# dontLoveBugs/CSPN_monodepth

Hardware: AMD Instinct MI355X
Metric: depth-maps/sec at 304x228 b=24, 24 CSPN iters (higher is better)
Workload: dtype f32

## Files before the change

### cspn_monodepth_amd/csrc/cspn_resident.hip

```cpp
#include "cspn_common.hpp"

#include <atomic>

namespace {

struct ResArgs {
    const float* g;
    long g_bs, g_cs;
    const float* d0;
    const float* sparse;
    float* out;
    float* xbuf;
    unsigned* flags;
    unsigned* status;
    unsigned* host_err;
    int last_chunk;
    unsigned seq;
    float* hist;
    float* w_out;
    float* s_out;
    const float* s_in;
    const float* target;
    double* macc;
    int nslots;
    int B, H, W, Wv, T, S;
    int tw, th, tiles_x, tiles_y;
    int wq, wr, hxw, hyw, dr, ls;
    int b0, nb;
    unsigned spin_limit;
    unsigned long long* dbg;
};

__device__ __forceinline__ void st4_dev(float* base, unsigned elem, float a, float b, float c, float d) {
    const v4f v = {a, b, c, d};
    asm volatile("global_store_dwordx4 %0, %1, %2 sc1" ::"v"(elem * 4u), "v"(v), "s"(base) : "memory");
}
template <typename T>
__device__ __forceinline__ T* uniform_ptr(T* p) {
    const unsigned long long u = reinterpret_cast<unsigned long long>(p);
    const unsigned lo = __builtin_amdgcn_readfirstlane((unsigned)u), hi = __builtin_amdgcn_readfirstlane((unsigned)(u >> 32));
    return reinterpret_cast<T*>(((unsigned long long)hi << 32) | lo);
}
#define GLB __attribute__((address_space(1)))
typedef GLB char* gptr;
__device__ __forceinline__ gptr at32(const float* base, unsigned e) {
    return (gptr) reinterpret_cast<unsigned long long>(base) + (e << 2);
}
__device__ __forceinline__ float4 ld4(gptr p) {
    const v4f v = *reinterpret_cast<const GLB v4f*>(p);
    return make_float4(v.x, v.y, v.z, v.w);
}
__device__ __forceinline__ float ld1(gptr p) { return *reinterpret_cast<const GLB float*>(p); }
__device__ __forceinline__ void st4(gptr p, float4 v) {
// ... 5 lines not shown
#endif
#ifndef CSPN_RES_STEP_PIPE
#define CSPN_RES_STEP_PIPE 0
#endif
#ifndef CSPN_RES_PUBLISH_ALL
#define CSPN_RES_PUBLISH_ALL 1
#endif
__device__ __forceinline__ void st4_hist(gptr p, float4 v) {
    const v4f w = {v.x, v.y, v.z, v.w};
    if (CSPN_RES_HIST_NT) __builtin_nontemporal_store(w, reinterpret_cast<GLB v4f*>(p));
    else *reinterpret_cast<GLB v4f*>(p) = w;
}
__device__ __forceinline__ float4 ld4_dev(gptr p) {
    const unsigned long long lo = __hip_atomic_load(reinterpret_cast<const GLB unsigned long long*>(p), __ATOMIC_RELAXED, __HIP_MEMORY_SCOPE_AGENT);
    const unsigned long long hi = __hip_atomic_load(reinterpret_cast<const GLB unsigned long long*>(p) + 1, __ATOMIC_RELAXED, __HIP_MEMORY_SCOPE_AGENT);
    return make_float4(__uint_as_float((unsigned)lo), __uint_as_float((unsigned)(lo >> 32)), __uint_as_float((unsigned)hi),
                       __uint_as_float((unsigned)(hi >> 32)));
}
__device__ __forceinline__ float ld1_dev(gptr p) {
    return __uint_as_float(__hip_atomic_load(reinterpret_cast<const GLB unsigned*>(p), __ATOMIC_RELAXED, __HIP_MEMORY_SCOPE_AGENT));
}

constexpr int RES_THREADS = 512;
constexpr int RES_PP = 16352;

template <int NQ, int NTHREADS, int BLEND, int MODE, int CLEAN, int PAC = 0>
__global__ __launch_bounds__(NTHREADS, NTHREADS / 256) void cspn3_resident(const ResArgs a) {
    static_assert(!PAC || MODE <= 2, "the softmax-weight form has no transposed sweep of its own (the published volume feeds MODE 3)");
    constexpr int R = 1, NT = 8, WIN = 6;
    constexpr bool SCORE = MODE == 1, TRANSG = MODE == 4, TRANS = MODE == 3 || TRANSG, HIST = MODE == 2 || TRANS;
    extern __shared__ __attribute__((aligned(16))) float lds[];
    __shared__ int wg_bad;

    const int tid = threadIdx.x;
    const int tiles_per_img = a.tiles_x * a.tiles_y;
    const int wg_round = a.nb * tiles_per_img;
    const int round = (int)blockIdx.x / wg_round;
    const int tile = xcd_contiguous_id((int)blockIdx.x - round * wg_round, wg_round);
    const int bl = tile / tiles_per_img;
    const int trem = tile - bl * tiles_per_img;
    const int ty = trem / a.tiles_x;
    const int tx = trem - ty * a.tiles_x;
    const int b = a.b0 + round * a.nb + bl;
    const int H = a.H, W = a.W;
    const int y0 = ty * a.th, x0 = tx * a.tw;
    const size_t HW = (size_t)H * W;
    const size_t plane = (size_t)a.B * HW;
    if (tid == 0) wg_bad = 0;
    int n_stamp = 0;
    auto stamp = [&]() { if (a.dbg && tid == 0 && round == 0 && n_stamp < 16) a.dbg[(size_t)blockIdx.x * 16 + n_stamp++] = wall_clock64(); };
    stamp();
    auto count_out = [&]() {
        if (HIST && tid == 0) {
            const unsigned old = __hip_atomic_fetch_add(a.status + 2, 1u, __ATOMIC_RELAXED, __HIP_MEMORY_SCOPE_AGENT);
            if (old + 1u == gridDim.x) {
                __hip_atomic_store(a.status + 2, 0u, __ATOMIC_RELAXED, __HIP_MEMORY_SCOPE_AGENT);
                if (a.host_err && a.last_chunk) __hip_atomic_store(a.host_err + 1, a.seq, __ATOMIC_RELAXED, __HIP_MEMORY_SCOPE_SYSTEM);
            }
        }
    };

    if (b >= a.B) { count_out(); return; }

    const float* __restrict__ din0 = uniform_ptr(a.d0 + (size_t)b * HW);
    const float* __restrict__ spg = BLEND ? uniform_ptr(a.sparse + (size_t)b * HW) : nullptr;

    const int wq = a.wq, wr = a.wr;
    const int sy = tid / wq;
    const int sx = tid - sy * wq;
    const int r0 = sy * NQ;
    const bool exch = a.T > a.S;
    const int rx0 = max(exch ? max(0, x0 - a.tw) : 0, min(x0 - a.hxw, W - 4 * wq));
    const int ry0 = max(exch ? max(0, y0 - a.th) : 0, min(y0 - a.hyw, H - wr));
    const int xq = rx0 + 4 * sx;
    const int yq0 = ry0 + r0;
    const bool x_in = (xq >= 0) && (xq < a.Wv);
    const int nval = a.Wv - xq;
    const int lane = tid & 63;
    const bool fix_left = (sx == 0) || (lane == 0);
    const bool fix_right = (sx == wq - 1) || (lane == 63);

    const int dr = a.dr, ls = a.ls;
    float* const cur = lds;
    float* const nxt = lds + RES_PP;
    const int yd0 = ry0 - R;
    const int xd0 = rx0 - 4;
    float4 st0[NQ + 1];
    unsigned st0_in = 0;
    const int step_r = NTHREADS / wq, step_q = NTHREADS - step_r * wq;
    {
    int row = sy, qx = sx;
#pragma unroll
    for (int u = 0; u <= NQ; ++u) {
        const int y = yd0 + row, x = xd0 + 4 + 4 * qx;
        const bool valid = row < dr;
        const bool in = valid && (y >= 0 && y < H && x >= 0 && x < a.Wv);
// ... 23 lines not shown
    float* const md_lds = lds + RES_PP + (size_t)a.dr * a.ls;
    const float* __restrict__ gq = uniform_ptr(a.g + (size_t)b * a.g_bs);
    float edge[NQ][6];
    const unsigned ucs = (unsigned)a.g_cs;
    float srow[TRANSG ? NQ + 2 : 1][6];
    if constexpr (TRANSG) {
        const float* __restrict__ sq = uniform_ptr(a.s_in + (size_t)b * HW);
#pragma unroll
        for (int m = 0; m < NQ + 2; ++m) {
            const int ys = yq0 - 1 + m;
            const bool v = x_in && ys >= 0 && ys < H;
            const unsigned o = v ? (unsigned)(ys * W + xq) : 0u;
            const float4 q4 = ld4(at32(sq, o));
            srow[m][0] = q4.x; srow[m][1] = q4.y; srow[m][2] = q4.z; srow[m][3] = q4.w;
            srow[m][4] = ld1(at32(sq, (v && fix_left && xq >= 1) ? o - 1u : 0u));
            srow[m][5] = ld1(at32(sq, (v && fix_right && xq + 4 < a.Wv) ? o + 4u : 0u));
        }
    }
#pragma unroll
    for (int i = 0; i < NQ; ++i) {
        const int r = r0 + i, y = yq0 + i;
        const bool ok = (r < wr) && x_in && (y >= 0) && (y < H);
        if (ok) in_img |= 1u << i;
        if (ok && y >= y0 && y < y0 + a.th && xq >= x0 && xq < x0 + a.tw) interior |= 1u << i;
        unsigned orow[3];
        bool rokv[3];
#pragma unroll
        for (int d = 0; d < 3; ++d) {
            const int row = y + d - 1;
            rokv[d] = ok && row >= 0 && row < H;
            orow[d] = rokv[d] ? (unsigned)(row * W + xq) : 0u;
        }
#pragma unroll
        for (int j = 0; j < NT; ++j) {
            const int lin = j < 4 ? j : j + 1;
            const int d = (PAC || TRANSG) ? 1 : lin / 3;
            const float4 v = ld4(at32(gq, (unsigned)((PAC || TRANSG) ? j : 7 - j) * ucs + orow[d]));
            wreg[i][j][0] = rokv[d] ? v.x : 0.f; wreg[i][j][1] = rokv[d] ? v.y : 0.f;
            wreg[i][j][2] = rokv[d] ? v.z : 0.f; wreg[i][j][3] = rokv[d] ? v.w : 0.f;
        }
#pragma unroll
        for (int t = 0; t < 6; ++t) edge[i][t] = 0.f;
        if (!PAC && !TRANSG && (fix_left || fix_right)) {
#pragma unroll
            for (int t = 0; t < 6; ++t) {
                const bool lft = t < 3;
                const int j = lft ? (t == 0 ? 0 : (t == 1 ? 3 : 5)) : (t == 3 ? 2 : (t == 4 ? 4 : 7));
// ... 148 lines not shown
        }
    }

    stamp();
    int r0L = r0, sxL = sx, yq0L = yq0, xqL = xq;
    asm volatile("" : "+v"(r0L), "+v"(sxL), "+v"(yq0L), "+v"(xqL));
    const bool active = (r0L < wr);
    const int cb = 4 + 4 * sxL;
    float* __restrict__ dout = HIST ? nullptr : uniform_ptr(a.out + (size_t)b * HW);
    float* hist_step = HIST ? uniform_ptr(a.hist + (size_t)b * HW) : nullptr;
    const int n_phase = (a.T + a.S - 1) / a.S;
    const int tile_global = b * tiles_per_img + trem;
    float own[NQ][4];
    float nbl[NQ], nbr[NQ];

    for (int p = 0; p < n_phase; ++p) {
        const int steps = (a.T - p * a.S) < a.S ? (a.T - p * a.S) : a.S;
        const bool last_phase = (p == n_phase - 1);
        const float* __restrict__ xin = uniform_ptr(a.xbuf + (size_t)((p + 1) & 1) * plane + (size_t)b * HW);
        if (p > 0) {
            int tidp = tid;
            asm volatile("" : "+v"(tidp));
            const int tq_in = min(a.tw, rx0 + 4 * wq - x0) >> 2;
            const int th_in = min(a.th, ry0 + wr - y0);
            const int nl = (x0 - rx0) >> 2;
            const int nside = wq - tq_in;
            const int nrow_t = (y0 - ry0) + R;
            const int n_top = nrow_t * wq;
            const int n_bot = (dr - nrow_t - th_in) * wq;
            const int n_side = th_in * nside;
            const int n_halo = n_top + n_bot + n_side;
            float ring_v = 0.f;
            int ring_at = -1;
            if (tidp < dr * 2 * R) {
                const int row = tidp / (2 * R), c = tidp - row * (2 * R);
                const int lc = (c < R) ? (4 - R + c) : (4 + 4 * wq + (c - R));
                const int y = yd0 + row, x = xd0 + lc;
                const bool in = (y >= 0 && y < H && x >= 0 && x < a.Wv);
                const float v = ld1_dev(at32(xin, in ? (unsigned)(y * W + x) : 0u));
                ring_v = in ? v : 0.f;
                ring_at = row * ls + lc;
            }
            for (int base = 0; base < n_halo; base += 2 * NTHREADS) {
                float4 hv[2];
                int at[2];
#pragma unroll
                for (int u = 0; u < 2; ++u) {
// ... 189 lines not shown
        stamp();
        const int plain_steps = last_phase ? steps - 1 : steps;
        using P0 = std::integral_constant<int, 0>;
        using P1 = std::integral_constant<int, 1>;
        if (__ballot(active) != 0ull) {
            int s = 0;
            for (; s + 1 < plain_steps; s += 2) {
                step(std::false_type{}, std::true_type{}, P0{}, 0);
                step(std::false_type{}, std::true_type{}, P1{}, 0);
            }
            if (s < plain_steps) step(std::false_type{}, std::true_type{}, P0{}, 0);
            if (last_phase) step(std::true_type{}, std::true_type{}, P0{}, plain_steps & 1);
        } else {
            for (int s = 0; s < plain_steps; ++s) step(std::false_type{}, std::false_type{}, P0{}, 0);
            if (last_phase) step(std::true_type{}, std::false_type{}, P0{}, 0);
        }
        stamp();
        if (!last_phase) {
            float* __restrict__ xout = uniform_ptr(a.xbuf + (size_t)(p & 1) * plane + (size_t)b * HW);
            if (active) {
                unsigned o0 = (unsigned)(yq0L * W + xqL);
                asm volatile("" : "+v"(o0));
#if !CSPN_RES_PUBLISH_ALL
                auto reg_x0 = [&](int t) { const int xx0 = t * a.tw; return max(max(0, xx0 - a.tw), min(xx0 - a.hxw, W - 4 * wq)); };
                auto reg_y0 = [&](int t) { const int yy0 = t * a.th; return max(max(0, yy0 - a.th), min(yy0 - a.hyw, H - wr)); };
                const int pubL = tx > 0 ? reg_x0(tx - 1) + 4 * wq + 1 : -(1 << 30);
                const int pubR = tx + 1 < a.tiles_x ? reg_x0(tx + 1) - 1 : (1 << 30);
                const int pubT = ty > 0 ? reg_y0(ty - 1) + wr + 1 : -(1 << 30);
                const int pubB = ty + 1 < a.tiles_y ? reg_y0(ty + 1) - 1 : (1 << 30);
                const bool col_read = (xqL < pubL) || (xqL + 3 >= pubR);
#endif
#pragma unroll
                for (int i = 0; i < NQ; ++i) {
#if !CSPN_RES_PUBLISH_ALL
                    const bool read = col_read || (yq0L + i < pubT) || (yq0L + i >= pubB);
#else
                    const bool read = true;
#endif
                    if (((interior >> i) & 1u) && read) st4_dev(xout, o0 + (unsigned)(i * W), own[i][0], own[i][1], own[i][2], own[i][3]);
                }
            }
            asm volatile("s_waitcnt vmcnt(0)" ::: "memory");
            __syncthreads();
            const unsigned want = a.seq + (unsigned)p + 1u;
            if (tid == 0) __hip_atomic_store(a.flags + tile_global, want, __ATOMIC_RELAXED, __HIP_MEMORY_SCOPE_AGENT);
            if (tid < 9 && tid != 4) {
                const int ny = ty + tid / 3 - 1, nx = tx + tid % 3 - 1;
                if (ny >= 0 && ny < a.tiles_y && nx >= 0 && nx < a.tiles_x) {
// ... 71 lines not shown
        }
        __syncthreads();
        if (tid < 10) {
            double v = 0.0;
            for (int w = 0; w < NTHREADS / 64; ++w) v += (double)part[w * 10 + tid];
            if (v != 0.0) atomicAdd(a.macc + (size_t)(blockIdx.x % a.nslots) * 10 + tid, v);
        }
    }
    count_out();
}

constexpr int RES_MAX_NQ = 5;

constexpr int RES_MAX_ROUNDS = 8;
#ifndef CSPN_RES_ONE_LAUNCH
#define CSPN_RES_ONE_LAUNCH 0
#endif
struct ResGeom {
    int S, tiles_x, tiles_y, tw, th, nq, wq, wr, hxw, hyw, dr, ls;
    int imgs_per_launch, launches;
    size_t lds_bytes;
    double cost;
    int threads = RES_THREADS;
};

int cu_count() {
    static std::atomic<int> cached[64];
    int dev = 0;
    if (hipGetDevice(&dev) != hipSuccess) return 0;
    int n = cached[dev & 63].load(std::memory_order_relaxed);
    if (n > 0) return n;
    hipDeviceProp_t prop;
    if (hipGetDeviceProperties(&prop, dev) != hipSuccess) return 0;
    cached[dev & 63].store(prop.multiProcessorCount, std::memory_order_relaxed);
    return prop.multiProcessorCount;
}

size_t res_lds_bytes(int dr, int ls, int nq, int blend, int threads = RES_THREADS) {
    return ((size_t)RES_PP + (size_t)dr * ls + (size_t)(blend ? 1 : 0) * threads * nq * 4 + 16 * 10) * sizeof(float);
}

#ifndef CSPN_RES_LS_SWIZZLE
#define CSPN_RES_LS_SWIZZLE 1
#endif
int res_row_stride(int wq, int nq, int dr) {
    const int lo = 4 * wq + 8;
    if (!CSPN_RES_LS_SWIZZLE) return lo;
    for (int cand = lo; cand < lo + 64; cand += 4)
        if ((((nq * cand - 4 * wq) % 64) + 64) % 64 == 0 && (size_t)dr * cand <= (size_t)RES_PP) return cand;
    return lo;
}

bool regions_inside_image(const ResGeom& g, int H, int W, int Wv, int T) {
    if (Wv != W) return false;
    const bool exch = T > g.S;
    for (int tx = 0; tx < g.tiles_x; ++tx) {
        const int x0 = tx * g.tw;
        int rx0 = x0 - g.hxw; if (rx0 > W - 4 * g.wq) rx0 = W - 4 * g.wq;
        int lo = exch ? x0 - g.tw : 0; if (lo < 0) lo = 0;
        if (rx0 < lo) rx0 = lo;
        if (rx0 + 4 * g.wq > W) return false;
    }
    for (int ty = 0; ty < g.tiles_y; ++ty) {
        const int y0 = ty * g.th;
        int ry0 = y0 - g.hyw; if (ry0 > H - g.wr) ry0 = H - g.wr;
        int lo = exch ? y0 - g.th : 0; if (lo < 0) lo = 0;
        if (ry0 < lo) ry0 = lo;
        if (ry0 + g.wr > H) return false;
    }
    return true;
}

bool resident_geometry(int B, int H, int W, int T, int blend, int ncu, int S_user, ResGeom* best, int threads = RES_THREADS) {
    if (W % 4 != 0 || ncu < 1 || T < 1) return false;
    if (threads != 1024) threads = RES_THREADS;
    const int max_nq = threads == 1024 ? 1 : RES_MAX_NQ;
    bool found = false;
    for (int S = (S_user > 0 ? S_user : 12); S >= (S_user > 0 ? S_user : 4); S -= (S > 8 ? 4 : 2)) {
        const int Se = S > T ? T : S;
        const int hyw = Se - 1, hxw = round_up4(Se - 1);
        const int phases = ceil_div(T, Se);
        if (phases > 1 && (Se & 1)) continue;
        for (int tx = 1; tx <= 32; ++tx) {
            const int tw = round_up4(ceil_div(W, tx));
            if (tx > 1 && (tw < 16 || ceil_div(W, tw) != tx)) continue;
            if (phases > 1 && tx > 1 && tw < 2 * hxw) continue;
            const int wq = (tw + 2 * hxw) / 4;
            if (wq > threads) continue;
            for (int ty = 1; ty <= 64; ++ty) {
                const int th = ceil_div(H, ty);
                if (ty > 1 && (th < 4 || ceil_div(H, th) != ty)) continue;
                if (phases > 1 && ty > 1 && th < 2 * hyw) continue;
                const int tiles = tx * ty;
                if (tiles > ncu) continue;
                const int wr = th + 2 * hyw;
                const int rows_per_thread_col = threads / wq;
                const int nq = ceil_div(wr, rows_per_thread_col);
                if (nq > max_nq) continue;
                const int dr = wr + 2, ls = res_row_stride(wq, nq, dr);
                if ((size_t)dr * ls > (size_t)RES_PP) continue;
                const size_t ldsb = res_lds_bytes(dr, ls, nq, blend, threads);
                if (ldsb > 160 * 1024) continue;
                int ipl = ncu / tiles;
                if (ipl > B) ipl = B;
                const int launches = ceil_div(B, ipl);
                ResGeom cand{Se, tx, ty, tw, th, nq, wq, wr, hxw, hyw, dr, ls, ipl, launches, ldsb, 0.0};
                const double pen = regions_inside_image(cand, H, W, W, T) ? 1.0 : 1.13;
                const double cost = launches * (8.0 + 2.0 * nq + T * (0.13 * nq + 0.1) * pen + (phases - 1) * (3.0 + 0.6 * nq));
                if (!found || cost < best->cost) {
                    found = true;
                    *best = ResGeom{Se, tx, ty, tw, th, nq, wq, wr, hxw, hyw, dr, ls, ipl, launches, ldsb, cost};
                    best->threads = threads;
                }
            }
        }
    }
    return found;
}

template <int NQ, int BLEND, int MODE, int CLEAN, int PAC = 0, int NTH = RES_THREADS>
int launch_resident_inst(const ResArgs& a, int grid, size_t lds_bytes, hipStream_t st) {
    constexpr auto kern = cspn3_resident<NQ, NTH, BLEND, MODE, CLEAN, PAC>;
    static std::atomic<size_t> granted[64];
    int dev = 0;
    HIP_OK(hipGetDevice(&dev));
    if (lds_bytes > 64 * 1024 && granted[dev & 63].load(std::memory_order_acquire) < lds_bytes) {
        HIP_OK(hipFuncSetAttribute(reinterpret_cast<const void*>(kern), hipFuncAttributeMaxDynamicSharedMemorySize, (int)lds_bytes));
        granted[dev & 63].store(lds_bytes, std::memory_order_release);
    }
    hipLaunchKernelGGL(kern, dim3(grid), dim3(NTH), lds_bytes, st, a);
    HIP_OK(hipGetLastError());
    return 1;
}

template <int CLEAN>
int launch_resident_1024(const ResArgs& a, int grid, size_t lds, int blend, int mode, hipStream_t st) {
    if (mode == 0) return blend ? launch_resident_inst<1, 1, 0, CLEAN, 0, 1024>(a, grid, lds, st) : launch_resident_inst<1, 0, 0, CLEAN, 0, 1024>(a, grid, lds, st);
    if (mode == 1) return blend ? launch_resident_inst<1, 1, 1, CLEAN, 0, 1024>(a, grid, lds, st) : launch_resident_inst<1, 0, 1, CLEAN, 0, 1024>(a, grid, lds, st);
    return fail("cspn3_forward_resident: 1024-thread workgroups serve the inference forms only");
}

template <int NQ, int CLEAN>
int launch_resident_c(const ResArgs& a, int grid, size_t lds, int blend, int mode, hipStream_t st) {
    if (mode >= 4 && mode <= 6) {
        if (mode == 6) return blend ? launch_resident_inst<NQ, 1, 2, CLEAN, 1>(a, grid, lds, st) : launch_resident_inst<NQ, 0, 2, CLEAN, 1>(a, grid, lds, st);
        if (blend) return mode == 5 ? launch_resident_inst<NQ, 1, 1, CLEAN, 1>(a, grid, lds, st) : launch_resident_inst<NQ, 1, 0, CLEAN, 1>(a, grid, lds, st);
        return mode == 5 ? launch_resident_inst<NQ, 0, 1, CLEAN, 1>(a, grid, lds, st) : launch_resident_inst<NQ, 0, 0, CLEAN, 1>(a, grid, lds, st);
    }
    if (mode == 7) return blend ? launch_resident_inst<NQ, 1, 4, CLEAN>(a, grid, lds, st) : launch_resident_inst<NQ, 0, 4, CLEAN>(a, grid, lds, st);
    if (mode == 3) return blend ? launch_resident_inst<NQ, 1, 3, CLEAN>(a, grid, lds, st) : launch_resident_inst<NQ, 0, 3, CLEAN>(a, grid, lds, st);
    if (blend) {
        if (mode == 2) return launch_resident_inst<NQ, 1, 2, CLEAN>(a, grid, lds, st);
        return mode ? launch_resident_inst<NQ, 1, 1, CLEAN>(a, grid, lds, st) : launch_resident_inst<NQ, 1, 0, CLEAN>(a, grid, lds, st);
    }
    if (mode == 2) return launch_resident_inst<NQ, 0, 2, CLEAN>(a, grid, lds, st);
    return mode ? launch_resident_inst<NQ, 0, 1, CLEAN>(a, grid, lds, st) : launch_resident_inst<NQ, 0, 0, CLEAN>(a, grid, lds, st);
}
template <int NQ>
int launch_resident_nq(const ResArgs& a, int grid, size_t lds, int blend, int mode, bool clean, hipStream_t st) {
    return clean ? launch_resident_c<NQ, 1>(a, grid, lds, blend, mode, st) : launch_resident_c<NQ, 0>(a, grid, lds, blend, mode, st);
}


}

namespace {
int resident_launch(const void* guidance, long bs, long cs, const void* d0, const void* sparse, void* out, void* history,
                    void* w8_out, float* s_out, void* work, unsigned seq, unsigned* host_err, int B, int H, int W, int W_valid,
                    int T, int blend, const void* target, double* acc, int nslots, const cspn_resident_plan* plan,
                    cspn_stream_t stream, bool transposed, bool pac = false, const float* s_in = nullptr);
}

extern "C" {

int cspn3_resident_plan(int B, int H, int W, int T, int blend, int n_cu, cspn_resident_plan* out) {
    if (!out || B < 1 || H < 1 || W < 1 || T < 0) return fail("cspn3_resident_plan: bad arguments");
    if (n_cu <= 0) n_cu = cu_count();
    if (n_cu <= 0) return fail("cspn3_resident_plan: no device (pass n_cu > 0 to plan without one)");
    ResGeom g;
    if (T < 1 || !resident_geometry(B, H, W, T, blend, n_cu, out->steps_per_phase, &g, out->threads))
        return fail("cspn3_resident_plan: no resident tiling for B=%d %dx%d T=%d on %d CUs (W %% 4 == 0 needed)", B, H, W, T, n_cu);
    if (ceil_div(T, g.S) > 255) return fail("cspn3_resident_plan: T=%d in %d-step phases is more than 255 phases", T, g.S);
    out->steps_per_phase = g.S; out->tiles_x = g.tiles_x; out->tiles_y = g.tiles_y; out->tile_w = g.tw; out->tile_h = g.th;
    out->quads_per_thread = g.nq; out->threads = g.threads; out->images_per_launch = g.imgs_per_launch;
    out->launches = g.launches; out->lds_bytes = (int)g.lds_bytes; out->n_cu = n_cu;
    out->region_over_tile = (float)((double)(4 * g.wq) * g.wr / ((double)g.tw * g.th));
    return 1;
}

size_t cspn3_resident_workspace_bytes(int B, int H, int W) {
    const size_t planes = (size_t)2 * B * H * W * sizeof(float);
    const size_t flags = ((size_t)B * (((size_t)H * W) / 16 + 1) + 4) * sizeof(unsigned);
    return ((planes + 15) & ~(size_t)15) + ((flags + 15) & ~(size_t)15);
}

int cspn3_forward_resident(const void* guidance, long bs, long cs, const void* d0, const void* sparse, void* out,
                           void* history, void* w8_out, float* s_out,
                           void* work, unsigned seq, unsigned* host_err, int B, int H, int W, int W_valid, int T, int blend,
                           const void* target, double* acc, int nslots, const cspn_resident_plan* plan,
                           cspn_stream_t stream) {
    return resident_launch(guidance, bs, cs, d0, sparse, out, history, w8_out, s_out, work, seq, host_err, B, H, W, W_valid, T,
                           blend, target, acc, nslots, plan, stream, false);
}

int cspn3_transposed_resident(const void* w8, const float* g_T, const float* sparse_f32, float* history, void* work,
                              unsigned seq, unsigned* host_err, int B, int H, int W, int W_valid, int T, int premask,
                              const cspn_resident_plan* plan, cspn_stream_t stream) {
    if (!w8 || !g_T || !history) return fail("cspn3_transposed_resident: bad arguments");
    if (premask && !sparse_f32) return fail("cspn3_transposed_resident: premask needs sparse");
// ... 36 lines not shown
        return fail("cspn3_forward_resident: bad arguments");
    if (!transposed && history && ((pac && !w8_out) || (!pac && !s_out) || target || acc || !aligned16(history) || (w8_out && !aligned16(w8_out)) || (s_out && !aligned16(s_out))))
        return fail("cspn3_forward_resident: the training form (history) needs s_out (w8_out is optional: null publishes S only), 16-byte aligned, and no scoring");
    if (!history && (w8_out || s_out)) return fail("cspn3_forward_resident: w8_out / s_out are outputs of the training form (history)");
    if (transposed && !aligned16(history)) return fail("cspn3_transposed_resident: history must be 16-byte aligned");
    if (blend != CSPN_BLEND_NONE && blend != CSPN_BLEND_SPARSE) return fail("cspn3_forward_resident: blend %d", blend);
    if (blend && !sparse) return fail("cspn3_forward_resident: blend needs sparse");
    if ((target || acc) && (!target || !acc || nslots < 1 || !aligned16(target)))
        return fail("cspn3_forward_resident: scoring needs target (16-byte aligned), acc and nslots >= 1");
    if ((W & 3) || (cs & 3) || (bs & 3)) return fail("cspn3_forward_resident: W and the guidance strides must be multiples of 4");
    if (cs < 0 || bs < 0 || cs >= (1L << 27) || (long)H * W >= (1L << 27))
        return fail("cspn3_forward_resident: images of >= 2^27 pixels / channel strides >= 2^27 elements are not supported (32-bit offsets)");
    if (!aligned16(guidance) || !aligned16(d0) || (out && !aligned16(out)) || !aligned16(work) || (sparse && !aligned16(sparse)))
        return fail("cspn3_forward_resident: tensors must be 16-byte aligned");
    if (W_valid < 0 || W_valid > W) return fail("cspn3_forward_resident: W_valid=%d outside (0, W=%d]", W_valid, W);
    if (seq == 0 || seq > 0x7fffff00u) return fail("cspn3_forward_resident: seq must be in [1, 2^31 - 256]");

    hipStream_t st = static_cast<hipStream_t>(stream);
    const int ncu = cu_count();
    if (ncu <= 0) return fail("cspn3_forward_resident: no device");
    ResGeom g;
    cspn_resident_plan rp{};
    if (plan) rp = *plan;
    if (rp.tiles_x > 0 && rp.tiles_y > 0 && rp.tile_w > 0 && rp.tile_h > 0 && rp.steps_per_phase > 0 && rp.images_per_launch > 0) {
        const int Se = rp.steps_per_phase > T ? T : rp.steps_per_phase;
        g.S = Se; g.tiles_x = rp.tiles_x; g.tiles_y = rp.tiles_y; g.tw = rp.tile_w; g.th = rp.tile_h;
        g.hyw = Se - 1; g.hxw = round_up4(Se - 1);
        g.wq = (g.tw + 2 * g.hxw) / 4; g.wr = g.th + 2 * g.hyw;
        g.dr = g.wr + 2;
        g.threads = rp.threads == 1024 ? 1024 : RES_THREADS;
        g.nq = g.wq > 0 && g.wq <= g.threads ? ceil_div(g.wr, g.threads / g.wq) : RES_MAX_NQ + 1;
        if (g.threads == 1024 && g.nq > 1) g.nq = RES_MAX_NQ + 1;
        g.ls = res_row_stride(g.wq, g.nq, g.dr);
        g.lds_bytes = res_lds_bytes(g.dr, g.ls, g.nq, blend, g.threads);
        g.imgs_per_launch = rp.images_per_launch;
        const int phases = ceil_div(T, Se);
        if ((g.tw & 3) || g.nq > RES_MAX_NQ || g.lds_bytes > 160 * 1024 || (size_t)g.dr * g.ls > (size_t)RES_PP || (phases > 1 && (Se & 1)) || g.tiles_x * g.tw < W || g.tiles_y * g.th < H ||
            (long)g.imgs_per_launch * g.tiles_x * g.tiles_y > ncu ||
            (phases > 1 && ((g.tiles_x > 1 && g.tw < 2 * g.hxw) || (g.tiles_y > 1 && g.th < 2 * g.hyw))))
            return fail("cspn3_forward_resident: the plan does not fit this problem / device (use cspn3_resident_plan)");
    } else if (!resident_geometry(B, H, W, T, blend, ncu, rp.steps_per_phase, &g, rp.threads)) {
        return fail("cspn3_forward_resident: no resident tiling for B=%d %dx%d T=%d", B, H, W, T);
    }
    if (ceil_div(T, g.S) > 255)
        return fail("cspn3_forward_resident: T=%d in %d-step phases is more than 255 phases (use the multi-launch schedule)", T, g.S);
    ResArgs a{};
    a.g = static_cast<const float*>(guidance); a.g_bs = bs; a.g_cs = cs;
    a.d0 = static_cast<const float*>(d0); a.sparse = static_cast<const float*>(sparse); a.out = static_cast<float*>(out);
    const size_t planes = (((size_t)2 * B * H * W * sizeof(float)) + 15) & ~(size_t)15;
    a.xbuf = static_cast<float*>(work);
    a.status = reinterpret_cast<unsigned*>(static_cast<char*>(work) + planes);
    a.flags = a.status + 4;
    if ((size_t)B * g.tiles_x * g.tiles_y > (size_t)B * (((size_t)H * W) / 16 + 1))
        return fail("cspn3_forward_resident: workspace too small for %d tiles", B * g.tiles_x * g.tiles_y);
    a.host_err = host_err;
    a.hist = static_cast<float*>(history); a.w_out = static_cast<float*>(w8_out); a.s_out = s_out;
    if (pac && transposed) return fail("cspn3_forward_resident: the softmax-weight form has no transposed sweep (use cspn3_transposed_resident on the volume)");
    const int mode = transposed ? (s_in ? 7 : 3) : (history ? 2 : (acc ? 1 : 0)) + (pac ? 4 : 0);
    a.s_in = s_in;
    a.seq = seq;
    a.target = static_cast<const float*>(target); a.macc = acc; a.nslots = nslots;
    a.B = B; a.H = H; a.W = W; a.Wv = (W_valid > 0 && W_valid < W) ? W_valid : W; a.T = T; a.S = g.S;
    a.tw = g.tw; a.th = g.th; a.tiles_x = g.tiles_x; a.tiles_y = g.tiles_y;
    a.wq = g.wq; a.wr = g.wr; a.hxw = g.hxw; a.hyw = g.hyw; a.dr = g.dr; a.ls = g.ls;
    a.spin_limit = rp.spin_limit ? rp.spin_limit : (4u << 20);
    a.dbg = rp.debug_stamps;
    const bool clean = regions_inside_image(g, H, W, a.Wv, T);
    if (rp.guard && ((mode != 0 && mode != 1 && mode != 2 && mode != 3 && mode != 7 && mode != 4 && mode != 6) || ((mode == 0 || mode == 1 || mode == 4) && !out) ||
                     !cspn_detail::resident_repair_fits(T)))
        return fail("cspn3_forward_resident: plan->guard serves inference (plain / scored), the training forward and the reverse sweeps, T <= 54 steps");
    const int ipl = g.imgs_per_launch < B ? g.imgs_per_launch : B;
    const int max_rounds = CSPN_RES_ONE_LAUNCH ? RES_MAX_ROUNDS : 1;
    for (int b0 = 0; b0 < B; b0 += ipl * max_rounds) {
        a.b0 = b0;
        a.nb = (B - b0) < ipl ? (B - b0) : ipl;
        const int rounds = ceil_div(B - b0, ipl) < max_rounds ? ceil_div(B - b0, ipl) : max_rounds;
        a.last_chunk = (b0 + ipl * max_rounds >= B) ? 1 : 0;
        const int grid = rounds * a.nb * g.tiles_x * g.tiles_y;
        int ok = 0;
        if (g.threads == 1024) {
            ok = clean ? launch_resident_1024<1>(a, grid, g.lds_bytes, blend, mode, st) : launch_resident_1024<0>(a, grid, g.lds_bytes, blend, mode, st);
            if (!ok) return 0;
            continue;
        }
        switch (g.nq) {
            case 1: ok = launch_resident_nq<1>(a, grid, g.lds_bytes, blend, mode, clean, st); break;
            case 2: ok = launch_resident_nq<2>(a, grid, g.lds_bytes, blend, mode, clean, st); break;
            case 3: ok = launch_resident_nq<3>(a, grid, g.lds_bytes, blend, mode, clean, st); break;
            case 4: ok = launch_resident_nq<4>(a, grid, g.lds_bytes, blend, mode, clean, st); break;
            case 5: ok = launch_resident_nq<5>(a, grid, g.lds_bytes, blend, mode, clean, st); break;
            default: return fail("cspn3_forward_resident: no instance for %d quads per thread", g.nq);
        }
        if (!ok) return 0;
    }
    if (rp.guard)
        return cspn_detail::resident_repair_launch(a.g, bs, cs, a.d0, a.sparse, a.out, a.hist, a.s_out, a.w_out, a.s_in,
                                                   mode == 7 ? 4 : mode == 4 ? 10 : mode == 6 ? 12 : mode, a.status, seq, B, H, W, a.Wv, T, blend ? 1 : 0, ncu, st,
                                                   a.target, a.macc, a.nslots);
    return 1;
}

}
// ... 1 lines not shown
```

### cspn_monodepth_amd/functional.py

```python
import ctypes
import math
import os
import threading
import weakref
import time

import torch

from . import _lib
from ._lib import BLEND_NONE, BLEND_PREMASK, BLEND_SPARSE, CSPN_F16, CSPN_F32, STEP_AUTO, STEP_DOT2, STEP_FMA, cspn_plan

_DEFAULT_PLANS = {}
_EVENT_LOG = None


class EventLog(list):

    def __init__(self, n_pairs=0, every=1):
        super(EventLog, self).__init__()
        self.every = max(1, int(every))
        self.calls = 0
        self.pool = []
        for _ in range(2 * int(n_pairs)):
            ev = torch.cuda.Event(enable_timing=True)
# ... 662 lines not shown

_RES_PLAN_CACHE = {}


def _resident_plan_cached(B, H, W, T, blend, dev):
    key = (B, H, W, T, blend, dev.index, _RESIDENT_MODE)
    hit = _RES_PLAN_CACHE.get(key)
    if hit is None:
        n_cu = _resident_state(dev)["n_cu"]
        if _RESIDENT_MODE == "on":
            rp = resident_plan(B, H, W, T, blend, n_cu)
        else:
            rp = None if _device_is_oversubscribed() else resident_pays(B, H, W, T, blend, dev)
        cp = None
        if rp is not None:
            cp = _lib.cspn_resident_plan()
            for name, _ in _lib.cspn_resident_plan._fields_:
                if name != "debug_stamps":
                    setattr(cp, name, rp[name])
        if len(_RES_PLAN_CACHE) > 1024:
            _RES_PLAN_CACHE.clear()
        hit = _RES_PLAN_CACHE[key] = (rp, cp)
    return hit


def resident_pays(B, H, W, T, blend, dev):
    rp = resident_plan(B, H, W, T, blend, _resident_state(dev)["n_cu"])
    if rp is None:
        return None
    if rp["region_over_tile"] > 3.6:
        return None
    return rp


def resident_supported(guidance, d0, sparse, T, plan=None, target=None):
    if _RESIDENT_MODE == "off" or plan is not None or _DEFAULT_PLANS.get(3) is not None or T < 1:
        return None
    if guidance.dtype != torch.float32 or d0.dtype != torch.float32 or not from_guidance_supported(guidance, d0, sparse, None):
        return None
    if target is not None and (target.dtype != torch.float32 or target.data_ptr() % 16):
        return None
    B, H, W = d0.shape
    if guidance.stride(1) >= (1 << 27) or H * W >= (1 << 27):
        return None
    return _resident_plan_cached(B, H, W, int(T), int(sparse is not None), guidance.device)[0]

# ... 258 lines not shown
    L = _lib.lib()
    hist = w8 = S_out = out = None
    if keep_history:
        hist = torch.empty((int(T), B, H, W), dtype=torch.float32, device=dev)
        w8 = torch.empty((B, 8, H, W), dtype=torch.float32, device=dev) if publish_weights else None
        S_out = torch.empty((B, H, W), dtype=torch.float32, device=dev)
    else:
        out = torch.empty((B, H, W), dtype=torch.float32, device=dev)
    tg, acc = score if score is not None else (None, None)
    rp = None
    if guard is None:
        guard = int(bool(_RESIDENT_GUARD) and (score is None or _RESIDENT_GUARD == "all") and int(T) <= _GUARD_MAX_T)
    guard = int(guard)
    if _plan is not None and not _RESIDENT_SPIN_LIMIT:
        rp = _plan
    elif steps_per_phase or spin_limit or debug_stamps is not None or threads:
        rp = _lib.cspn_resident_plan()
        rp.steps_per_phase = int(steps_per_phase)
        rp.threads = int(threads)
        rp.spin_limit = int(spin_limit)
        rp.debug_stamps = None if debug_stamps is None else debug_stamps.data_ptr()
        rp.guard = guard
    else:
        rp = _with_spin_limit(_resident_plan_cached(B, H, W, int(T), int(blend), dev)[1], guard=guard)
    def launch(work, seq, host_err_ptr, stream_ptr):
        return L.cspn3_forward_resident(_p(guidance), guidance.stride(0), guidance.stride(1), _p(d0), _p(sparse), _p(out),
                                        _p(hist), _p(w8), _p(S_out), _p(work), seq, host_err_ptr, B, H, W, int(valid_w),
                                        int(T), int(blend), _p(tg), _p(acc), 0 if acc is None else int(acc.shape[0]),
                                        None if rp is None else ctypes.byref(rp), stream_ptr)

    redo = None
    if not keep_history:
        scored = score is not None

        def redo(out, guidance, d0, sparse, tg):
            from . import evaluation
            tgp = None if tg is None else tg.reshape(B, H, W)
            if scored:
                _unscore_failed_launch(out, tgp, acc)
            res, _ = propagate_from_guidance(guidance, d0.reshape(B, H, W), None if sparse is None else sparse.reshape(B, H, W), T, blend,
                                             valid_w=valid_w)
            out.copy_(res)
            if scored:
                evaluation.metric_sums(out, tgp, out=acc)

    ok = _resident_launch(dev, B, H, W, int(T), launch, reports_done=bool(keep_history), redo=redo,
                          out=hist[int(T) - 1] if keep_history else out, inputs=() if keep_history else (guidance, d0, sparse, tg),
# ... 540 lines not shown
            if out is None:
                with torch.no_grad():
                    out = forward_resident(guidance, blur_depth, sparse_depth, prop_time, fast_plan.blend, score=(target, acc),
                                           _plan=fast_plan.plan if _RESIDENT_GUARD != "all" else None)
            return out.unsqueeze(1)
    dev = _require_device(guidance, blur_depth, sparse_depth, target)
    W0 = guidance.shape[-1]
    pad = _row_padding(W0, plan)
    if pad:
        guidance, blur_depth, sparse_depth, target = (_pad_w(t, pad) for t in (guidance[:, :8], blur_depth, sparse_depth,
                                                                               target))
    vw = W0 if pad else 0
    B, C, H, W = guidance.shape
    d0 = _plane(blur_depth, B, H, W, "blur_depth")
    sp = _plane(sparse_depth, B, H, W, "sparse_depth")
    tg = _plane(target, B, H, W, "target")
    blend = BLEND_SPARSE if sp is not None else BLEND_NONE
    with torch.no_grad():
        if guidance.dtype == d0.dtype == tg.dtype and resident_supported(guidance, d0, sp, prop_time, plan, tg) is not None:
            out = forward_resident(guidance, d0, sp, prop_time, blend, score=(tg, acc), valid_w=vw)
            if key is not None and not pad and blur_depth.dim() == 4 and target.dim() == 4 and (sparse_depth is None or sparse_depth.dim() == 4):
                if len(_SCORED_FAST) > 256:
                    _SCORED_FAST.clear()
                _SCORED_FAST[key] = _ScoredFast(_resident_plan_cached(B, H, W, int(prop_time), int(blend), guidance.device)[1], guidance,
                                                prop_time, blend, acc)
            return out.unsqueeze(1)[..., :W0]
        if (_FROM_GUIDANCE and from_guidance_supported(guidance, d0, sp, plan) and guidance.dtype == d0.dtype
                and tg.dtype == d0.dtype and tg.data_ptr() % 16 == 0):
            p = resolve_plan(3, B, H, W, prop_time, False, plan)
            if (prop_time > p["steps_per_launch"] and not p["force_scalar"]
                    and (p["quads_per_thread"], p["threads"]) in _SCORED_INSTANCES[3]):
                out, _ = propagate_from_guidance(guidance, d0, sp, prop_time, blend, plan=plan, score=(tg, acc),
                                                 valid_w=vw)
                return out.unsqueeze(1)[..., :W0]
        w8, _, _ = cspn3_prepare(guidance, valid_w=vw)
        if scored_supported(w8, d0, sp, tg, 3, prop_time, plan):
            out = propagate_scored(w8, d0, sp, 3, prop_time, blend, tg, acc, plan, valid_w=vw)
        else:
            out, _ = propagate(w8, d0, sp, 3, prop_time, blend, plan=plan, valid_w=vw)
            evaluation.metric_sums(out, tg, out=acc)
    del dev
    return out.unsqueeze(1)[..., :W0]


def pac_refine_and_score(x, guided, sparse_depth, target, acc, prop_time=24, plan=None, state_dtype=None):
    from . import evaluation
    _require_device(x, guided, sparse_depth, target)
# ... 68 lines not shown
```

Baseline: 524,500.

## Add 768-thread clipped resident tiling with uneven edge row tiles for scored path

Adds a 768-thread resident kernel variant whose vertical tiles have uneven heights: the first and last tiles are sized so their halo regions stay inside the image, avoiding out-of-image rows. A new geometry search picks tile counts and heights under this scheme, and the scored inference path switches to it when the 512-thread plan needs more than three quads per thread and still fits in one launch. The aim is less redundant halo work and fewer per-thread quads. In exchange it adds a separate planner, a new kernel instantiation, and more complex tile-boundary arithmetic for halo publishing.

```diff
diff --git a/cspn_monodepth_amd/csrc/cspn_resident.hip b/cspn_monodepth_amd/csrc/cspn_resident.hip
--- a/cspn_monodepth_amd/csrc/cspn_resident.hip
+++ b/cspn_monodepth_amd/csrc/cspn_resident.hip
@@ -29,6 +29,7 @@
     int b0, nb;
     unsigned spin_limit;
     unsigned long long* dbg;
+    int th0, thl;
 };
 
 __device__ __forceinline__ void st4_dev(float* base, unsigned elem, float a, float b, float c, float d) {
@@ -80,6 +81,28 @@
 }
 
 constexpr int RES_THREADS = 512;
+constexpr int RES_THREADS_CLIPPED = 768;
+
+template <bool UNEVEN = true>
+__host__ __device__ __forceinline__ int res_row_y0(int ty, int th0, int th) {
+    if (!UNEVEN) return ty * th;
+    return ty <= 0 ? 0 : th0 + (ty - 1) * th;
+}
+template <bool UNEVEN = true>
+__host__ __device__ __forceinline__ int res_row_h(int ty, int tiles_y, int th0, int th, int thl) {
+    if (!UNEVEN) return th;
+    return ty == 0 ? th0 : (ty == tiles_y - 1 ? thl : th);
+}
+__host__ __device__ __forceinline__ int res_region_x0(int tx, int tw, int hxw, int wq, int W, bool exch) {
+    const int x0 = tx * tw;
+    return max(exch ? max(0, x0 - tw) : 0, min(x0 - hxw, W - 4 * wq));
+}
+template <bool UNEVEN = true>
+__host__ __device__ __forceinline__ int res_region_y0(int ty, int th0, int th, int hyw, int wr, int H, bool exch) {
+    const int y0 = res_row_y0<UNEVEN>(ty, th0, th);
+    const int lo = exch ? (UNEVEN ? res_row_y0(ty - 1, th0, th) : max(0, y0 - th)) : 0;
+    return max(lo, min(y0 - hyw, H - wr));
+}
 constexpr int RES_PP = 16352;
 
 template <int NQ, int NTHREADS, int BLEND, int MODE, int CLEAN, int PAC = 0>
@@ -101,7 +124,9 @@
     const int tx = trem - ty * a.tiles_x;
     const int b = a.b0 + round * a.nb + bl;
     const int H = a.H, W = a.W;
-    const int y0 = ty * a.th, x0 = tx * a.tw;
+    constexpr bool UNEVEN = NTHREADS == RES_THREADS_CLIPPED;
+    const int y0 = res_row_y0<UNEVEN>(ty, a.th0, a.th), x0 = tx * a.tw;
+    const int th_t = res_row_h<UNEVEN>(ty, a.tiles_y, a.th0, a.th, a.thl);
     const size_t HW = (size_t)H * W;
     const size_t plane = (size_t)a.B * HW;
     if (tid == 0) wg_bad = 0;
@@ -128,8 +153,8 @@
     const int sx = tid - sy * wq;
     const int r0 = sy * NQ;
     const bool exch = a.T > a.S;
-    const int rx0 = max(exch ? max(0, x0 - a.tw) : 0, min(x0 - a.hxw, W - 4 * wq));
-    const int ry0 = max(exch ? max(0, y0 - a.th) : 0, min(y0 - a.hyw, H - wr));
+    const int rx0 = res_region_x0(tx, a.tw, a.hxw, wq, W, exch);
+    const int ry0 = res_region_y0<UNEVEN>(ty, a.th0, a.th, a.hyw, wr, H, exch);
     const int xq = rx0 + 4 * sx;
     const int yq0 = ry0 + r0;
     const bool x_in = (xq >= 0) && (xq < a.Wv);
@@ -199,7 +224,7 @@
         const int r = r0 + i, y = yq0 + i;
         const bool ok = (r < wr) && x_in && (y >= 0) && (y < H);
         if (ok) in_img |= 1u << i;
-        if (ok && y >= y0 && y < y0 + a.th && xq >= x0 && xq < x0 + a.tw) interior |= 1u << i;
+        if (ok && y >= y0 && y < y0 + th_t && xq >= x0 && xq < x0 + a.tw) interior |= 1u << i;
         unsigned orow[3];
         bool rokv[3];
 #pragma unroll
@@ -394,7 +419,7 @@
             int tidp = tid;
             asm volatile("" : "+v"(tidp));
             const int tq_in = min(a.tw, rx0 + 4 * wq - x0) >> 2;
-            const int th_in = min(a.th, ry0 + wr - y0);
+            const int th_in = min(th_t, ry0 + wr - y0);
             const int nl = (x0 - rx0) >> 2;
             const int nside = wq - tq_in;
             const int nrow_t = (y0 - ry0) + R;
@@ -630,8 +655,8 @@
                 unsigned o0 = (unsigned)(yq0L * W + xqL);
                 asm volatile("" : "+v"(o0));
 #if !CSPN_RES_PUBLISH_ALL
-                auto reg_x0 = [&](int t) { const int xx0 = t * a.tw; return max(max(0, xx0 - a.tw), min(xx0 - a.hxw, W - 4 * wq)); };
-                auto reg_y0 = [&](int t) { const int yy0 = t * a.th; return max(max(0, yy0 - a.th), min(yy0 - a.hyw, H - wr)); };
+                auto reg_x0 = [&](int t) { return res_region_x0(t, a.tw, a.hxw, wq, W, true); };
+                auto reg_y0 = [&](int t) { return res_region_y0<UNEVEN>(t, a.th0, a.th, a.hyw, wr, H, true); };
                 const int pubL = tx > 0 ? reg_x0(tx - 1) + 4 * wq + 1 : -(1 << 30);
                 const int pubR = tx + 1 < a.tiles_x ? reg_x0(tx + 1) - 1 : (1 << 30);
                 const int pubT = ty > 0 ? reg_y0(ty - 1) + wr + 1 : -(1 << 30);
@@ -749,7 +774,9 @@
     size_t lds_bytes;
     double cost;
     int threads = RES_THREADS;
+    int th0 = 0, thl = 0;
 };
+void set_uniform_rows(ResGeom* g) { g->th0 = g->thl = g->th; }
 
 int cu_count() {
     static std::atomic<int> cached[64];
@@ -782,23 +809,76 @@
     if (Wv != W) return false;
     const bool exch = T > g.S;
     for (int tx = 0; tx < g.tiles_x; ++tx) {
-        const int x0 = tx * g.tw;
-        int rx0 = x0 - g.hxw; if (rx0 > W - 4 * g.wq) rx0 = W - 4 * g.wq;
-        int lo = exch ? x0 - g.tw : 0; if (lo < 0) lo = 0;
-        if (rx0 < lo) rx0 = lo;
-        if (rx0 + 4 * g.wq > W) return false;
+        const int rx0 = res_region_x0(tx, g.tw, g.hxw, g.wq, W, exch);
+        if (rx0 < 0 || rx0 + 4 * g.wq > W) return false;
     }
     for (int ty = 0; ty < g.tiles_y; ++ty) {
-        const int y0 = ty * g.th;
-        int ry0 = y0 - g.hyw; if (ry0 > H - g.wr) ry0 = H - g.wr;
-        int lo = exch ? y0 - g.th : 0; if (lo < 0) lo = 0;
-        if (ry0 < lo) ry0 = lo;
-        if (ry0 + g.wr > H) return false;
+        const int ry0 = res_region_y0(ty, g.th0, g.th, g.hyw, g.wr, H, exch);
+        if (ry0 < 0 || ry0 + g.wr > H) return false;
     }
     return true;
 }
 
+bool clipped_geometry(int H, int W, int T, int Se, int tiles_x, int tiles_y, int tw, int th0, int blend, ResGeom* g) {
+    if (tiles_x < 1 || tiles_y < 1 || tw < 4 || (tw & 3) || th0 < 1 || Se < 1) return false;
+    const int hyw = Se - 1, hxw = round_up4(Se - 1), phases = ceil_div(T, Se);
+    if (phases > 1 && (Se & 1)) return false;
+    if (tiles_x * tw < W || (tiles_x - 1) * tw >= W) return false;
+    if (phases > 1 && tiles_x > 1 && tw < 2 * hxw) return false;
+    int th = th0, thl = th0, wr = H;
+    if (tiles_y == 1) {
+        if (th0 < H) return false;
+        th = thl = th0 = H;
+    } else {
+        wr = th0 + hyw;
+        th = wr - 2 * hyw;
+        thl = H - th0 - (tiles_y - 2) * th;
+        if (th < 1 || thl < 1 || thl > th0) return false;
+        if (phases > 1 && (th0 < 2 * hyw || (tiles_y > 2 && th < 2 * hyw) || thl < hyw)) return false;
+    }
+    int wx = 0;
+    for (int tx = 0; tx < tiles_x; ++tx) {
+        const int lo = tx * tw - hxw > 0 ? tx * tw - hxw : 0, hi = (tx + 1) * tw + hxw < W ? (tx + 1) * tw + hxw : W;
+        if (hi - lo > wx) wx = hi - lo;
+    }
+    const int wq = wx / 4;
+    if (wq < 1 || ceil_div(wr, 3) * wq > RES_THREADS_CLIPPED) return false;
+    const int dr = wr + 2, ls = res_row_stride(wq, 3, dr);
+    if ((size_t)dr * ls > (size_t)RES_PP) return false;
+    const size_t ldsb = res_lds_bytes(dr, ls, 3, blend, RES_THREADS_CLIPPED);
+    if (ldsb > 160 * 1024) return false;
+    *g = ResGeom{Se, tiles_x, tiles_y, tw, th, 3, wq, wr, hxw, hyw, dr, ls, 0, 0, ldsb, 0.0};
+    g->threads = RES_THREADS_CLIPPED; g->th0 = th0; g->thl = thl;
+    return regions_inside_image(*g, H, W, W, T);
+}
+
+bool resident_geometry_clipped(int B, int H, int W, int T, int blend, int ncu, int S_user, ResGeom* best) {
+    if (W % 4 != 0 || ncu < 1 || T < 1) return false;
+    bool found = false;
+    for (int S = (S_user > 0 ? S_user : 12); S >= (S_user > 0 ? S_user : 4); S -= (S > 8 ? 4 : 2)) {
+        const int Se = S > T ? T : S;
+        const int hyw = Se - 1, phases = ceil_div(T, Se);
+        for (int tx = 1; tx <= 32; ++tx) {
+            const int tw = round_up4(ceil_div(W, tx));
+            if (tx > 1 && (tw < 16 || ceil_div(W, tw) != tx)) continue;
+            for (int ty = 1; ty <= 64 && tx * ty <= ncu; ++ty) {
+                const int wr = ty == 1 ? H : ceil_div(H + 2 * hyw * (ty - 1), ty);
+                ResGeom cand;
+                if (!clipped_geometry(H, W, T, Se, tx, ty, tw, ty == 1 ? H : wr - hyw, blend, &cand)) continue;
+                int ipl = ncu / (tx * ty);
+                if (ipl > B) ipl = B;
+                cand.imgs_per_launch = ipl; cand.launches = ceil_div(B, ipl);
+                const double q = (double)cand.wq * cand.wr / 256.0 / 3.0;
+                cand.cost = cand.launches * (8.0 + 2.0 * q + T * (0.13 * q + 0.1) + (phases - 1) * (3.0 + 0.6 * q));
+                if (!found || cand.cost < best->cost) { found = true; *best = cand; }
+            }
+        }
+    }
+    return found;
+}
+
 bool resident_geometry(int B, int H, int W, int T, int blend, int ncu, int S_user, ResGeom* best, int threads = RES_THREADS) {
+    if (threads == RES_THREADS_CLIPPED) return resident_geometry_clipped(B, H, W, T, blend, ncu, S_user, best);
     if (W % 4 != 0 || ncu < 1 || T < 1) return false;
     if (threads != 1024) threads = RES_THREADS;
     const int max_nq = threads == 1024 ? 1 : RES_MAX_NQ;
@@ -832,12 +912,14 @@
                 if (ipl > B) ipl = B;
                 const int launches = ceil_div(B, ipl);
                 ResGeom cand{Se, tx, ty, tw, th, nq, wq, wr, hxw, hyw, dr, ls, ipl, launches, ldsb, 0.0};
+                set_uniform_rows(&cand);
                 const double pen = regions_inside_image(cand, H, W, W, T) ? 1.0 : 1.13;
                 const double cost = launches * (8.0 + 2.0 * nq + T * (0.13 * nq + 0.1) * pen + (phases - 1) * (3.0 + 0.6 * nq));
                 if (!found || cost < best->cost) {
                     found = true;
                     *best = ResGeom{Se, tx, ty, tw, th, nq, wq, wr, hxw, hyw, dr, ls, ipl, launches, ldsb, cost};
                     best->threads = threads;
+                    set_uniform_rows(best);
                 }
             }
         }
@@ -867,6 +949,12 @@
     return fail("cspn3_forward_resident: 1024-thread workgroups serve the inference forms only");
 }
 
+int launch_resident_768(const ResArgs& a, int grid, size_t lds, int blend, int mode, hipStream_t st) {
+    if (mode == 0) return blend ? launch_resident_inst<3, 1, 0, 1, 0, RES_THREADS_CLIPPED>(a, grid, lds, st) : launch_resident_inst<3, 0, 0, 1, 0, RES_THREADS_CLIPPED>(a, grid, lds, st);
+    if (mode == 1) return blend ? launch_resident_inst<3, 1, 1, 1, 0, RES_THREADS_CLIPPED>(a, grid, lds, st) : launch_resident_inst<3, 0, 1, 1, 0, RES_THREADS_CLIPPED>(a, grid, lds, st);
+    return fail("cspn3_forward_resident: 768-thread workgroups serve the inference forms only");
+}
+
 template <int NQ, int CLEAN>
 int launch_resident_c(const ResArgs& a, int grid, size_t lds, int blend, int mode, hipStream_t st) {
     if (mode >= 4 && mode <= 6) {
@@ -908,10 +996,13 @@
     if (T < 1 || !resident_geometry(B, H, W, T, blend, n_cu, out->steps_per_phase, &g, out->threads))
         return fail("cspn3_resident_plan: no resident tiling for B=%d %dx%d T=%d on %d CUs (W %% 4 == 0 needed)", B, H, W, T, n_cu);
     if (ceil_div(T, g.S) > 255) return fail("cspn3_resident_plan: T=%d in %d-step phases is more than 255 phases", T, g.S);
-    out->steps_per_phase = g.S; out->tiles_x = g.tiles_x; out->tiles_y = g.tiles_y; out->tile_w = g.tw; out->tile_h = g.th;
+    out->steps_per_phase = g.S; out->tiles_x = g.tiles_x; out->tiles_y = g.tiles_y; out->tile_w = g.tw;
+    out->tile_h = g.threads == RES_THREADS_CLIPPED ? g.th0 : g.th;
     out->quads_per_thread = g.nq; out->threads = g.threads; out->images_per_launch = g.imgs_per_launch;
     out->launches = g.launches; out->lds_bytes = (int)g.lds_bytes; out->n_cu = n_cu;
-    out->region_over_tile = (float)((double)(4 * g.wq) * g.wr / ((double)g.tw * g.th));
+    out->region_over_tile = g.threads == RES_THREADS_CLIPPED
+        ? (float)((double)(4 * g.wq) * g.wr * g.tiles_x * g.tiles_y / ((double)H * W))
+        : (float)((double)(4 * g.wq) * g.wr / ((double)g.tw * g.th));
     return 1;
 }
 
@@ -994,12 +1085,23 @@
     ResGeom g;
     cspn_resident_plan rp{};
     if (plan) rp = *plan;
-    if (rp.tiles_x > 0 && rp.tiles_y > 0 && rp.tile_w > 0 && rp.tile_h > 0 && rp.steps_per_phase > 0 && rp.images_per_launch > 0) {
+    const int Wv = (W_valid > 0 && W_valid < W) ? W_valid : W;
+    if (rp.threads == RES_THREADS_CLIPPED && (transposed || history || pac || Wv != W)) {
+        rp.threads = RES_THREADS;
+        rp.tiles_x = rp.tiles_y = rp.tile_w = rp.tile_h = rp.images_per_launch = 0;
+    }
+    if (rp.threads == RES_THREADS_CLIPPED && rp.tiles_x > 0 && rp.tiles_y > 0 && rp.tile_w > 0 && rp.tile_h > 0 && rp.steps_per_phase > 0 && rp.images_per_launch > 0) {
+        if (!clipped_geometry(H, W, T, rp.steps_per_phase > T ? T : rp.steps_per_phase, rp.tiles_x, rp.tiles_y, rp.tile_w, rp.tile_h, blend, &g) ||
+            (long)rp.images_per_launch * g.tiles_x * g.tiles_y > ncu)
+            return fail("cspn3_forward_resident: the clipped plan does not fit this problem / device (use cspn3_resident_plan)");
+        g.imgs_per_launch = rp.images_per_launch;
+    } else if (rp.tiles_x > 0 && rp.tiles_y > 0 && rp.tile_w > 0 && rp.tile_h > 0 && rp.steps_per_phase > 0 && rp.images_per_launch > 0) {
         const int Se = rp.steps_per_phase > T ? T : rp.steps_per_phase;
         g.S = Se; g.tiles_x = rp.tiles_x; g.tiles_y = rp.tiles_y; g.tw = rp.tile_w; g.th = rp.tile_h;
         g.hyw = Se - 1; g.hxw = round_up4(Se - 1);
         g.wq = (g.tw + 2 * g.hxw) / 4; g.wr = g.th + 2 * g.hyw;
         g.dr = g.wr + 2;
+        set_uniform_rows(&g);
         g.threads = rp.threads == 1024 ? 1024 : RES_THREADS;
         g.nq = g.wq > 0 && g.wq <= g.threads ? ceil_div(g.wr, g.threads / g.wq) : RES_MAX_NQ + 1;
         if (g.threads == 1024 && g.nq > 1) g.nq = RES_MAX_NQ + 1;
@@ -1032,8 +1134,8 @@
     a.s_in = s_in;
     a.seq = seq;
     a.target = static_cast<const float*>(target); a.macc = acc; a.nslots = nslots;
-    a.B = B; a.H = H; a.W = W; a.Wv = (W_valid > 0 && W_valid < W) ? W_valid : W; a.T = T; a.S = g.S;
-    a.tw = g.tw; a.th = g.th; a.tiles_x = g.tiles_x; a.tiles_y = g.tiles_y;
+    a.B = B; a.H = H; a.W = W; a.Wv = Wv; a.T = T; a.S = g.S;
+    a.tw = g.tw; a.th = g.th; a.tiles_x = g.tiles_x; a.tiles_y = g.tiles_y; a.th0 = g.th0; a.thl = g.thl;
     a.wq = g.wq; a.wr = g.wr; a.hxw = g.hxw; a.hyw = g.hyw; a.dr = g.dr; a.ls = g.ls;
     a.spin_limit = rp.spin_limit ? rp.spin_limit : (4u << 20);
     a.dbg = rp.debug_stamps;
@@ -1050,6 +1152,11 @@
         a.last_chunk = (b0 + ipl * max_rounds >= B) ? 1 : 0;
         const int grid = rounds * a.nb * g.tiles_x * g.tiles_y;
         int ok = 0;
+        if (g.threads == RES_THREADS_CLIPPED) {
+            if (!clean) return fail("cspn3_forward_resident: a clipped plan whose regions leave the image");
+            if (!launch_resident_768(a, grid, g.lds_bytes, blend, mode, st)) return 0;
+            continue;
+        }
         if (g.threads == 1024) {
             ok = clean ? launch_resident_1024<1>(a, grid, g.lds_bytes, blend, mode, st) : launch_resident_1024<0>(a, grid, g.lds_bytes, blend, mode, st);
             if (!ok) return 0;
diff --git a/cspn_monodepth_amd/functional.py b/cspn_monodepth_amd/functional.py
--- a/cspn_monodepth_amd/functional.py
+++ b/cspn_monodepth_amd/functional.py
@@ -708,6 +708,29 @@
             _RES_PLAN_CACHE.clear()
         hit = _RES_PLAN_CACHE[key] = (rp, cp)
     return hit
+
+
+_RES_SCORED_PLAN_CACHE = {}
+_CLIPPED_SCORED = os.environ.get("CSPN_RESIDENT_CLIPPED", "1") != "0"
+
+
+def _scored_plan(cp, B, H, W, T, blend, dev):
+    if cp is None or not _CLIPPED_SCORED or cp.launches != 1 or cp.quads_per_thread <= 3 or cp.threads != 512:
+        return cp
+    key = (id(cp), B, H, W, T, blend)
+    hit = _RES_SCORED_PLAN_CACHE.get(key)
+    if hit is None or hit[0] is not cp:
+        rp = resident_plan(B, H, W, T, blend, _resident_state(dev)["n_cu"], threads=768)
+        c2 = cp
+        if rp is not None and rp["launches"] == 1 and rp["steps_per_phase"] == cp.steps_per_phase:
+            c2 = _lib.cspn_resident_plan()
+            for name, _ in _lib.cspn_resident_plan._fields_:
+                if name != "debug_stamps":
+                    setattr(c2, name, rp[name])
+        if len(_RES_SCORED_PLAN_CACHE) > 256:
+            _RES_SCORED_PLAN_CACHE.clear()
+        hit = _RES_SCORED_PLAN_CACHE[key] = (cp, c2)
+    return hit[1]
 
 
 def resident_pays(B, H, W, T, blend, dev):
@@ -1012,7 +1035,10 @@
         rp.debug_stamps = None if debug_stamps is None else debug_stamps.data_ptr()
         rp.guard = guard
     else:
-        rp = _with_spin_limit(_resident_plan_cached(B, H, W, int(T), int(blend), dev)[1], guard=guard)
+        cp = _resident_plan_cached(B, H, W, int(T), int(blend), dev)[1]
+        if score is not None and not keep_history and not valid_w:
+            cp = _scored_plan(cp, B, H, W, int(T), int(blend), dev)
+        rp = _with_spin_limit(cp, guard=guard)
     def launch(work, seq, host_err_ptr, stream_ptr):
         return L.cspn3_forward_resident(_p(guidance), guidance.stride(0), guidance.stride(1), _p(d0), _p(sparse), _p(out),
                                         _p(hist), _p(w8), _p(S_out), _p(work), seq, host_err_ptr, B, H, W, int(valid_w),
@@ -1599,7 +1625,8 @@
             if key is not None and not pad and blur_depth.dim() == 4 and target.dim() == 4 and (sparse_depth is None or sparse_depth.dim() == 4):
                 if len(_SCORED_FAST) > 256:
                     _SCORED_FAST.clear()
-                _SCORED_FAST[key] = _ScoredFast(_resident_plan_cached(B, H, W, int(prop_time), int(blend), guidance.device)[1], guidance,
+                _SCORED_FAST[key] = _ScoredFast(_scored_plan(_resident_plan_cached(B, H, W, int(prop_time), int(blend), guidance.device)[1],
+                                                             B, H, W, int(prop_time), int(blend), guidance.device), guidance,
                                                 prop_time, blend, acc)
             return out.unsqueeze(1)[..., :W0]
         if (_FROM_GUIDANCE and from_guidance_supported(guidance, d0, sp, plan) and guidance.dtype == d0.dtype
```

Result: faster. 572,800, median of 6 (+9.2%).
